# RobertPincus/i3rc-monte-carlo-model

Measured on AMD Instinct MI355X. Metric: photons/s (whole node) + achieved HBM GB/s, I3RC step-cloud 1e8 photons, higher is better.
Workload: dtype f32

## Files before the change

i3rc-monte-carlo-model_amd/binding.py:

```python
import ctypes as C
import os

import numpy as np

from . import build as _build

fp = C.POINTER(C.c_float)
dp = C.POINTER(C.c_double)
ip = C.POINTER(C.c_int32)
lp = C.POINTER(C.c_int64)
up = C.POINTER(C.c_uint32)

MAX_COMPONENTS = 255
MAX_DIRECTIONS = 255
NUM_COUNTERS = 16
COUNTER_NAMES = ["photons", "dropped", "cellSteps", "scatterings", "surfaceHits", "exitsTop", "roulette",
                 "shadowSteps", "tracerCalls", "rngDraws", "raysSkipped"]

SYMBOLS = [
    "i3rc_hip_create", "i3rc_hip_destroy", "i3rc_hip_last_error", "i3rc_hip_set_inverse_table",
    "i3rc_hip_set_forward_tables", "i3rc_hip_set_params", "i3rc_hip_set_surface", "i3rc_hip_set_directions",
    "i3rc_hip_get_tally_layout", "i3rc_hip_bind_tally_buffer", "i3rc_hip_set_stream", "i3rc_hip_use_own_stream", "i3rc_hip_zero_tallies",
    "i3rc_hip_launch_batch", "i3rc_hip_run_batches", "i3rc_hip_run_batches_moments", "i3rc_hip_get_moments_layout", "i3rc_hip_compute_batch", "i3rc_hip_expect_batches", "i3rc_hip_run_replay", "i3rc_hip_trace_rays", "i3rc_hip_synchronize",
    "i3rc_hip_fetch_tallies", "i3rc_hip_normalise", "i3rc_hip_last_kernel_ms", "i3rc_hip_kernel_ms_history", "i3rc_hip_set_tuning", "i3rc_hip_force_general_kernel", "i3rc_hip_select_kernel", "i3rc_hip_set_light_threshold", "i3rc_hip_set_launch_limit",
    "i3rc_hip_set_batch_fusion", "i3rc_hip_select_grid_place", "i3rc_hip_has_column_records", "i3rc_hip_column_records", "i3rc_hip_column_records_base", "i3rc_hip_lds_plan", "i3rc_hip_lds_plan_words", "i3rc_hip_set_lds_tallies", "i3rc_hip_last_kernel_name", "i3rc_hip_last_plan", "i3rc_hip_timed_launch_count", "i3rc_hip_philox_blocks", "i3rc_hip_arith_check", "i3rc_hip_find_index", "i3rc_hip_surface_reflectance", "i3rc_hip_device_count", "i3rc_hip_version",
    "i3rc_hip_set_level_fluxes", "i3rc_hip_get_level_flux_layout", "i3rc_hip_normalise_level_fluxes",
    "i3rc_hip_set_actinic_flux", "i3rc_hip_get_actinic_flux_layout", "i3rc_hip_normalise_actinic_flux",
    "i3rc_hip_set_path_lengths", "i3rc_hip_get_path_length_layout", "i3rc_hip_normalise_path_lengths",
    "i3rc_hip_set_path_histogram", "i3rc_hip_get_path_histogram_layout", "i3rc_hip_normalise_path_histogram",
    "i3rc_hip_problem_facts", "i3rc_hip_plan_launch",
    "i3rc_hip_run_batches_diagnostic_moments", "i3rc_hip_get_diagnostic_moments_layout", "i3rc_hip_diagnostic_moments_layout_words",
    "i3rc_hip_set_path_spectrum", "i3rc_hip_get_path_moments_layout", "i3rc_hip_path_moments_layout_words", "i3rc_hip_run_batches_path_moments",
]


class Params(C.Structure):
    _fields_ = [
        ("surfaceAlbedo", C.c_float), ("useSurfaceBDRF", C.c_int32), ("useRayTracing", C.c_int32),
        ("useRussianRoulette", C.c_int32), ("useHybridPhaseFunsForIntenCalcs", C.c_int32),
# ... 151 lines not shown
    L.i3rc_hip_fetch_tallies.argtypes = [H, dp]
    L.i3rc_hip_normalise.argtypes = [H, dp, fp, fp, fp, fp, fp, fp]
    L.i3rc_hip_last_kernel_ms.argtypes = [H, fp]
    L.i3rc_hip_kernel_ms_history.argtypes = [H, C.c_int, fp]
    if hasattr(L, "i3rc_hip_last_kernel_name"):
        L.i3rc_hip_last_kernel_name.argtypes = [H]
        L.i3rc_hip_timed_launch_count.argtypes = [H]
        L.i3rc_hip_timed_launch_count.restype = C.c_int64
        L.i3rc_hip_last_kernel_name.restype = C.c_char_p
    if hasattr(L, "i3rc_hip_last_plan"):
        L.i3rc_hip_last_plan.argtypes = [H, ip, C.c_int]
    L.i3rc_hip_set_tuning.argtypes = [H, C.c_int, C.c_int]
    L.i3rc_hip_force_general_kernel.argtypes = [H, C.c_int]
    L.i3rc_hip_select_kernel.argtypes = [H, C.c_int]
    L.i3rc_hip_set_light_threshold.argtypes = [H, C.c_int]
    L.i3rc_hip_set_launch_limit.argtypes = [H, C.c_int64]
    if hasattr(L, "i3rc_hip_set_batch_fusion"):
        L.i3rc_hip_set_batch_fusion.argtypes = [H, C.c_int]
    if hasattr(L, "i3rc_hip_select_grid_place"):
        L.i3rc_hip_select_grid_place.argtypes = [H, C.c_int]
        L.i3rc_hip_has_column_records.argtypes = [H]
        L.i3rc_hip_column_records.argtypes = [C.c_int, C.c_int, C.c_int, fp, up]
    if hasattr(L, "i3rc_hip_column_records_base"):
        L.i3rc_hip_column_records_base.argtypes = [C.c_int, C.c_int, C.c_int, fp, up, fp]
    if hasattr(L, "i3rc_hip_lds_plan"):
        L.i3rc_hip_lds_plan.argtypes = [ip, ip]
        L.i3rc_hip_set_lds_tallies.argtypes = [H, C.c_int]
    if hasattr(L, "i3rc_hip_lds_plan_words"):
        L.i3rc_hip_lds_plan_words.argtypes = [ip, C.c_int, ip, C.c_int]
    L.i3rc_hip_philox_blocks.argtypes = [H, C.c_uint32, C.c_uint32, C.c_int64, C.c_int64, C.c_int, up, fp]
# ... 45 lines not shown
```

i3rc-monte-carlo-model_amd/csrc/i3rc_hip.hip:

```cpp
#include "../../include/i3rc_hip.h"

#include <hip/hip_runtime.h>
#include <ctime>
#include <map>
#include <utility>

#include "kernels.hpp"
#include "tally_block.hpp"
#include "launch_plan.hpp"

using namespace i3rc;

namespace {

thread_local std::string g_createError;

bool poison() { static const bool on = std::getenv("I3RC_POISON") != nullptr; return on; }

bool tracing() { static const bool on = std::getenv("I3RC_TRACE") != nullptr; return on; }
double trace_ms() {
  timespec ts; clock_gettime(CLOCK_MONOTONIC, &ts);
  static const double t0 = ts.tv_sec * 1e3 + ts.tv_nsec * 1e-6;
  return ts.tv_sec * 1e3 + ts.tv_nsec * 1e-6 - t0;
}


struct DevBuf {
  void *p = nullptr;
  size_t bytes = 0;
  DevBuf() = default;
  DevBuf(const DevBuf &) = delete;
  DevBuf &operator=(const DevBuf &) = delete;
  ~DevBuf() { if (p) (void)hipFree(p); }
  hipError_t upload(const void *src, size_t n) {
    hipError_t e = alloc(n);
    if (e != hipSuccess) return e;
    if (n) e = hipMemcpy(p, src, n, hipMemcpyHostToDevice);
    return e;
  }
  hipError_t alloc(size_t n) {
    if (p) { (void)hipFree(p); p = nullptr; }
    bytes = n;
    hipError_t e = hipMalloc(&p, n ? n : 4);
    if (e == hipSuccess && poison()) {
      e = hipMemset(p, 0xFF, n ? n : 4);
      if (e == hipSuccess) e = hipDeviceSynchronize();
    }
    return e;
  }
};

}

struct i3rc_hip_integrator : ProblemFacts {
  int device = 0;
  std::vector<float> xE, yE, zE;
  std::vector<double> areaFrac, layerDepth;
  DevBuf dxE, dyE, dzE, dExt, dCum, dSsa, dPf;
  DevBuf dCellRec;
  DevBuf dExtBrick;
  DevBuf dClearMap;
  DevBuf dColRec;
  DevBuf dColBase;
  bool compDirty = true;
  std::vector<DevBuf> dInv, dInvCos, dFwd, dFwdOrig;
  DevBuf dComp;
  DevBuf dXs, dYs, dBrdf;
  float brdf0 = 0.f;
  DevBuf dDir;
  DevBuf dBins;
  std::vector<float> binEdges;

  i3rc_tally_layout layout{};
  TallyView view{};
  DevBuf ownTally;
  double *tally = nullptr;
  DevBuf workCounter;
  DevBuf srcBuf[5];

  struct PipeSlot {
    hipStream_t stream = nullptr;
    DevBuf tally, counter, excess;
    double *pinned = nullptr;
    hipEvent_t done = nullptr;
// ... 522 lines not shown
  int64_t *const out[4] = {binUp, binPathUp, binDown, binPathDown};
  for (int f = 0; f < 4; ++f)
    if (out[f]) *out[f] = on ? block + path_bin_field(f, h->pathBins) : -1;
  if (nBins) *nBins = on ? h->pathBins : 0;
  if (total) *total = h->layout.total;
  return 0;
}

int i3rc_hip_set_tuning(i3rc_hip_integrator *h, int evThreshold, int blocksPerCU) {
  if (!h) return 1;
  drop_lookahead(h);
  if (evThreshold >= 0 && evThreshold <= 64) h->evThreshold = evThreshold;
  if (blocksPerCU >= 0 && blocksPerCU <= 8) h->blocksPerCU = blocksPerCU;
  return 0;
}

int i3rc_hip_set_light_threshold(i3rc_hip_integrator *h, int lanes) {
  if (!h) return 1;
  drop_lookahead(h);
  if (lanes < 0 || lanes > 64) return h->fail("i3rc_hip_set_light_threshold: need 1..64 lanes (0 = default)");
  h->lightThreshold = lanes;
  return 0;
}

int i3rc_hip_set_launch_limit(i3rc_hip_integrator *h, int64_t photons) {
  if (!h) return 1;
  drop_lookahead(h);
  if (photons < 0) return h->fail("i3rc_hip_set_launch_limit: negative limit");
  h->launchLimit = photons;
  return 0;
// ... 128 lines not shown
  std::memset(&P, 0, sizeof(P));
  P.nx = h->nx; P.ny = h->ny; P.nz = h->nz; P.ncomp = h->ncomp;
  P.xyRegular = h->xyRegular; P.zRegular = h->zRegular;
  P.x0 = h->xE.front(); P.xMax = h->xE.back();
  P.y0 = h->yE.front(); P.yMax = h->yE.back();
  P.z0 = h->zE.front(); P.zMax = h->zE.back();
  P.deltaX = h->xE[1] - h->xE[0]; P.deltaY = h->yE[1] - h->yE[0]; P.deltaZ = h->zE[1] - h->zE[0];
  P.xE = (const float *)h->dxE.p; P.yE = (const float *)h->dyE.p; P.zE = (const float *)h->dzE.p;
  P.colRec = (const uint2 *)h->dColRec.p; P.colBase = (const float *)h->dColBase.p;
  P.extBrick = (const float *)h->dExtBrick.p;
  P.bsx = h->bsx; P.bsy = h->bsy; P.bsz = h->bsz; P.nbx = h->nbx; P.nbxy = h->nbx * h->nby;
  P.clearMap = (const uint32_t *)h->dClearMap.p; P.clearShift = h->clearShift; P.clearNx = h->clearNx;
  P.totalExt = (const float *)h->dExt.p;
}

int make_problem(i3rc_hip_integrator *h, const LaunchDecision &d, DevProblem &P, hipStream_t stream, double *tally) {
  fill_geometry(h, P);
  if (d.place != GRID_COLUMNS && d.place != GRID_COLBASE) P.colRec = nullptr;
  if (d.place != GRID_COLBASE) P.colBase = nullptr;
  if (d.place != GRID_BRICKS) P.extBrick = nullptr;
  P.cumExt = (const float *)h->dCum.p; P.ssa = (const float *)h->dSsa.p;
  P.pfIndex = (const int32_t *)h->dPf.p;
  P.cellRec = (const uint4 *)h->dCellRec.p;
  if (h->compDirty) {
    if (hipStreamSynchronize(stream) != hipSuccess ||
        hipMemcpy(h->dComp.p, h->comp.data(), sizeof(CompTables) * h->ncomp, hipMemcpyHostToDevice) != hipSuccess)
      return h->fail("copying the component table descriptors failed");
    h->compDirty = false;
  }
  P.comp = (const CompTables *)h->dComp.p;
  P.comp0 = h->comp[0];
// ... 4 lines not shown
  P.useRayTracing = traced(*h) ? 1 : 0; P.useRR = h->params.useRussianRoulette;
  P.nDir = h->nDir; P.useHybrid = h->params.useHybridPhaseFunsForIntenCalcs;
  P.numOrdersOrig = h->params.numOrdersOrigPhaseFunIntenCalcs; P.useRRI = h->params.useRussianRouletteForIntensity;
  P.limitContrib = h->params.limitIntensityContributions; P.zetaMin = h->params.zetaMin;
  P.maxContrib = h->params.maxIntensityContribution; P.maxExt = h->maxExt;
  P.dirCos = (const float *)h->dDir.p;
  if (h->extra == EXTRA_PATH_BINS && h->nDir == 0) P.dirCos = (const float *)h->dBins.p;
  P.uniformSsa = h->uniformSsa; P.uniformPf = h->uniformPf;
  P.eventFlags = event_flags(P.uniformSsa, P.uniformPf, P.useBDRF != 0, P.albedo, P.useRR != 0);
  P.tally = tally;
  const TallyView &V = h->view;
  P.oUp = (int)V.fluxUp; P.oDown = (int)V.fluxDown; P.oAbs = (int)V.fluxAbsorbed; P.oVol = (int)V.volumeAbsorption;
  P.oInt = (int)V.intensityByComponent; P.oExc = (int)V.intensityExcess; P.oCnt = (int)V.counters;
  P.rayQueueCap = d.rayQueueCap;
  P.ldsTallies = d.ldsTallies; P.ldsVolume = d.ldsVolume; P.ldsIntensity = d.ldsIntensity; P.ldsGrid = d.ldsGrid | (d.ldsBins ? kLdsGridBinSums : 0);
  return 0;
}

__global__ void __launch_bounds__(256) absorbed_columns_kernel(double *blocks, long long stride, int oAbs, int oVol, int ncol, int nz) {
  const int col = (int)(blockIdx.x * 256 + threadIdx.x);
  if (col >= ncol) return;
  double *const blk = blocks + (size_t)blockIdx.y * stride;
  double s = 0.0;
  for (int k = 0; k < nz; ++k) s += blk[oVol + (size_t)k * ncol + col];
  blk[oAbs + col] = s;
}
int absorbed_columns(i3rc_hip_integrator *h, hipStream_t stream, double *blocks, int nBlocks, long long stride) {
  if (!h->absorbing || nBlocks < 1) return 0;
  const int ncol = h->nx * h->ny;
  for (int first = 0; first < nBlocks; first += 65535) {
    const int n = std::min(65535, nBlocks - first);
// ... 23 lines not shown
  for (int k = 0; k < 5; ++k) if (!arrs[k]) return h->fail("explicit photon stream: null array");
  for (int64_t i = 0; i < n; ++i) {
    const float mu = src->mu[i];
    if (!(std::fabs(mu) <= 1.f) || !(std::fabs(mu) > FLT_MIN)) return h->fail("setIllumination: solarMu out of bounds");
    if (!(src->x[i] >= 0.f && src->x[i] <= 1.f) || !(src->y[i] >= 0.f && src->y[i] <= 1.f) || !(src->z[i] >= 0.f && src->z[i] <= 1.f))
      return h->fail("setIllumination: photon position out of bounds (relative positions lie in [0, 1])");
    if (!std::isfinite(src->phi[i])) return h->fail("setIllumination: solarAzimuth out of bounds");
  }
  for (int k = 0; k < 5; ++k) {
    HIPCHK(h, h->srcBuf[k].upload(arrs[k], sizeof(float) * (size_t)n));
    *dst[k] = (const float *)h->srcBuf[k].p;
  }
  return 0;
}

int prepare_launch(i3rc_hip_integrator *h, const StreamKind &s, const i3rc_source *src, int64_t n, hipStream_t stream, double *tally,
                   Launch &L, RunArgs &A) {
  L.d = plan_launch(*h, EnvKnobs::process(), {s, src->kind});
  if (!L.d.refusal.empty() && L.d.early) return h->fail(L.d.refusal);
  if (upload_source(h, src, n, A)) return 1;
  if (!L.d.refusal.empty()) return h->fail(L.d.refusal);
  return make_problem(h, L.d, L.P, stream, tally);
}

using Kernel = void (*)(DevProblem, RunArgs, int, int);
struct KernelEntry {
  KernelKey key;
  Kernel fn;
  const char *name;
};

template <class Rng>
constexpr const char *rng_name() {
  if constexpr (Rng::kExtra == EXTRA_LEVELS) return "PhiloxLevelStream";
  else if constexpr (Rng::kExtra == EXTRA_TRACKS) return "PhiloxTrackStream";
  else if constexpr (Rng::kExtra == EXTRA_PATHS) return "PhiloxPathStream";
  else if constexpr (Rng::kExtra == EXTRA_PATH_BINS) return "PhiloxBinStream";
// ... 132 lines not shown
        int tx = 1, ty = 8;
        for (int cx = 2; cx <= 8; cx *= 2)
          if ((double)h->nx / cx + (double)h->ny / (8 / cx) < (double)h->nx / tx + (double)h->ny / ty) { tx = cx; ty = 8 / cx; }
        hipLaunchKernelGGL(slab_count_kernel, dim3(kSlabSortBlocks), dim3(256), 0, stream, A.seed0, A.seed1, A.firstPhoton, A.nPhotons, span,
                           tx, ty, (unsigned *)sb.blockCounts.p);
        hipLaunchKernelGGL(slab_scan_kernel, dim3(1), dim3(8), 0, stream, (int)kSlabSortBlocks, (const unsigned *)sb.blockCounts.p,
                           (SlabMeta *)sb.meta.p, (unsigned *)sb.blockBase.p);
        hipLaunchKernelGGL(slab_fill_kernel, dim3(kSlabSortBlocks), dim3(256), 0, stream, A.seed0, A.seed1, A.firstPhoton, A.nPhotons, span,
                           tx, ty, (const unsigned *)sb.blockBase.p, (uint32_t *)sb.ids.p);
        HIPCHK(h, hipGetLastError());
        B.slabIds = (const uint32_t *)sb.ids.p; B.slabMeta = (SlabMeta *)sb.meta.p;
      }
    }
    static const long long chunkMax = std::max(64ll, env_int("I3RC_CHUNK_MAX", 256));
    B.chunk = (int)std::min<long long>(chunkMax, std::max<long long>(64, A.nPhotons / (blocks * (threads / 64) * 8)));
    HIPCHK(h, hipMemsetAsync(A.workCounter, 0, sizeof(unsigned long long), stream));
    return 0;
  });
  if (rc) return 1;
  return absorbed_columns(h, stream, L.P.tally, 1, 0);
}

__global__ void __launch_bounds__(256) reduce_replicas_kernel(const double *blocks, double *out, long long nBlocksOut, int R, long long stride) {
  const long long i = (long long)blockIdx.x * 256 + threadIdx.x;
  if (i >= nBlocksOut * stride) return;
  const long long b = i / stride, e = i - b * stride;
  const double *src = blocks + (size_t)b * R * stride + e;
  double v = 0.0;
  for (int r = 0; r < R; ++r) v += src[(size_t)r * stride];
  out[i] = v;
// ... 1073 lines not shown
```

i3rc-monte-carlo-model_amd/csrc/kernels.hpp:

```cpp
#pragma once
#include <cstddef>
#include "tally_block.hpp"
#include "event_flags.hpp"
#include "pass_decision.hpp"
#include "tracer.hpp"
#include "tuning.hpp"

namespace i3rc {

enum LaneState { ST_TRACE = 0, ST_EVENT = 1, ST_DROPPED = 2, ST_NEW = 3, ST_DONE = 4,
                 ST_EXIT = 5 };

struct WaveCounters {
  uint32_t photons = 0, dropped = 0, steps = 0, scat = 0, surf = 0, top = 0, roul = 0, shadow = 0, calls = 0;
};
struct NestedCounters { uint32_t shadow = 0, calls = 0; };
struct LanePairs {
  uint32_t word = 0u;
  __device__ __forceinline__ void add(bool low, bool high) { word += (low ? 1u : 0u) + (high ? 1u << 16 : 0u); }
  __device__ __forceinline__ uint32_t low() const { return word & 0xffffu; }
  __device__ __forceinline__ uint32_t high() const { return word >> 16; }
  static __device__ __forceinline__ bool about_to_overflow(LanePairs a, LanePairs b) { return ((a.word | b.word) & ((1u << 15) | (1u << 31))) != 0u; }
};

// ... 336 lines not shown
};
template <class Rng>
constexpr bool has_start_store(bool intensity, bool general, int grid, bool multi) {
  return !Rng::kReplay && !Rng::kBatched && Rng::kExtra == EXTRA_NONE && !intensity && !general && !multi && grid != GRID_BRICKS;
}
template <class Rng, bool INTENSITY, bool GENERAL, int GRID, bool TBL = false, bool DIRECT = false, bool MULTI = false>
__global__ void __launch_bounds__(TBL ? 1024 : 256, (planned_waves<Rng, INTENSITY, GENERAL, GRID, TBL, MULTI>()))
photon_kernel(const DevProblem P, const RunArgs A, const int evThreshold, const int lightThreshold) {
  extern __shared__ __attribute__((aligned(16))) float smem[];
  Lds L;
  constexpr bool STORE = has_start_store<Rng>(INTENSITY, GENERAL, GRID, MULTI);
  constexpr bool FLAGS = STORE && I3RC_EVENT_FLAGS != 0;
  constexpr int STEP_FORM = !STORE ? 0 : (I3RC_STEP_BIASED_ADDRESS ? STEP_BIASED : 0) | (I3RC_STEP_STATE_SELECTS ? STEP_MASKS : 0) |
                                         (I3RC_STEP_COLD_ERROR ? STEP_COLD_ERROR : 0) | (I3RC_STEP_ADVANCE_MASKS ? STEP_ADVANCE_MASKS : 0);
  constexpr bool ROULETTE_BIT = FLAGS && I3RC_ROULETTE_FLAG != 0;
  constexpr bool PASS_BITS = STORE && I3RC_PASS_DECISION != 0;
  constexpr bool TURN_WORD = STORE && I3RC_TURN_ALL_WORD != 0;
  constexpr bool TURN_RANGE = STORE && I3RC_TURN_STATE_RANGE != 0;
  constexpr int kStDropped = TURN_RANGE ? (int)ST_DONE : (int)ST_DROPPED, kStDone = TURN_RANGE ? (int)ST_DROPPED : (int)ST_DONE;
  static_assert(!TURN_RANGE || (ST_NEW == 3 && kStDropped == 4 && ST_EXIT == 5 && kStDone < ST_NEW && ST_TRACE < ST_NEW && ST_EVENT < ST_NEW),
                "the turnover states are the states from ST_NEW on");
  constexpr bool CHAIN = !GENERAL && Rng::kBatched && INTENSITY && !DIRECT && GRID == GRID_BRICKS;
  constexpr bool ZERO_IS_SLOW = GENERAL || CHAIN;
  lds_float *startSlots = nullptr;
  constexpr bool TRACK = Rng::kExtra == EXTRA_TRACKS;
  lds_f64 *trackSums = nullptr;
  constexpr bool BINS = Rng::kExtra == EXTRA_PATH_BINS;
  BinTable bins;
  {
    const LdsPlan lp = lds_plan(P, INTENSITY && !Rng::kReplay, DIRECT, GRID, INTENSITY, TBL ? 16 : 4, 0, STORE);
// ... 228 lines not shown
      uint32_t draws = rng.take_used();
#pragma unroll
      for (int off = 32; off > 0; off >>= 1) draws += (uint32_t)__shfl_xor((int)draws, off, 64);
      if ((threadIdx.x & 63) == 0) {
        double *const c = counter_block(res.batch);
        const uint32_t v[8] = {wc.steps, wc.scat, wc.surf, wc.top, wc.roul, wc.shadow, wc.scat + wc.surf + wc.top + wc.calls, draws};
        const int at[8] = {I3RC_CNT_CELL_STEPS, I3RC_CNT_SCATTERINGS, I3RC_CNT_SURFACE_HITS, I3RC_CNT_EXITS_TOP, I3RC_CNT_ROULETTE,
                           I3RC_CNT_SHADOW_STEPS, I3RC_CNT_TRACER_CALLS, I3RC_CNT_RNG_DRAWS};
#pragma unroll
        for (int k = 0; k < 8; ++k)
          if (v[k] != 0u) unsafeAtomicAdd(c + at[k], (double)v[k]);
        if (raysSkipped != 0u) unsafeAtomicAdd(c + I3RC_CNT_RAYS_SKIPPED, (double)raysSkipped);
      }
      raysSkipped = 0u;
    }
    if (!BATCHED && (threadIdx.x & 63) == 0) {
      const uint32_t calls = STORE ? wc.scat + wc.surf + wc.top + wc.dropped : wc.calls;
      const uint32_t c[9] = {wc.photons, wc.dropped, wc.steps, wc.scat, wc.surf, wc.top, wc.roul, wc.shadow, calls};
      const ColdArgs ka = cold_args();
      double *const counters = ka->P.tally + ka->P.oCnt;
#pragma unroll
      for (int k = 0; k < 9; ++k)
        if (c[k] != 0u) unsafeAtomicAdd(counters + k, (double)c[k]);
    }
    wc = WaveCounters();
  };
  auto make_ray = [&](const auto &Px, const auto &Ax, int info, float inX, float inY, float inZ, uint32_t photonLo, uint32_t photonHi,
                      uint32_t eventBlock, uint32_t batch, int dIdx, float &rayWord, float &normOut, float &tauFreeOut, float &targetOut) -> bool {
    const int comp = EventInfo::component(info);
    const float uz = L.dirCos[3 * dIdx + 2];
    float norm;
    if (comp < 1) norm = 1.0f / kPi;
    else {
// ... 344 lines not shown
          }
          if constexpr (LANE_COUNTS) {
            const bool leaves = isNew && mine >= 0 && mineBatch != rng.batch && (accSteps | accA.word | accB.word | rng.used) != 0u;
            if (__ballot(leaves) != 0ull) flush_lanes(leaves);
          }
          if (isNew) {
            if (mine < 0) st = kStDone;
            else rng.start((uint64_t)(Ae.firstPhoton + mine), mineBatch);
          }
        }
      } else if constexpr (STORE) {
        if (newMask != 0ull) {
          int need = __popcll(newMask);
          int rank = lanes_below(newMask);
          long long mine = -1;
          for (;;) {
            const int take = need < startAvail ? need : startAvail;
            if (isNew && mine < 0 && rank >= 0 && rank < take) {
              mine = res.next - startAvail + rank;
              const StartSlot::Words s = StartSlot::load(startSlots + kStartWords * ((unsigned)mine & (unsigned)(kStartSlots - 1)));
              r.x = s.x; r.y = s.y; r.ix = s.ix; r.iy = s.iy; r.target = s.depth;
            }
            startAvail -= take;
            wc.photons += (unsigned)take;
            need -= take; rank -= take;
            if (need == 0) break;
            long long end = startState.end();
            if (res.next >= end) {
              if (end >= cold_args()->A.nPhotons) break;
              const unsigned refilled = (unsigned)__builtin_amdgcn_readfirstlane(startState.w[WaveStartState::kRefills]) + 1u;
              startState.w[WaveStartState::kRefills] = (int)refilled;
              if ((refilled & 3u) == 0u || wc.steps > 0x40000000u) flush_counters();
              else adapt_thresholds();
              res.refill();
              end = res.end;
              startState.save_end(end);
              if (res.next >= end) break;
            }
            const long long left = end - res.next;
            const int n = left < (long long)kStartSlots ? (int)left : kStartSlots;
            {
              const long long i = res.next + (long long)(threadIdx.x & 63);
              const Philox4 o = rng.first_block_of((uint64_t)(cold_args()->A.firstPhoton + i));
              const float px = u32_to_unit_float(o.v[0]);
              float py = u32_to_unit_float(o.v[1]);
#ifdef I3RC_EXPERIMENT_SLAB
              py *= 0.125f;
// ... 5 lines not shown
                const auto &Px = cold_args()->P;
                x = Px.x0 + px * (Px.xMax - Px.x0);
                ci = min((int)exact_div(x - Px.x0, Px.deltaX, refined_rcp(Px.deltaX)) + 1, Px.nx);
                if (fabsf(L.xE[ci] - x) < spacingf(x)) ci = ci + 1;
                ci = ci == Px.nx + 1 ? 1 : ci;
              }
              {
                const auto &Py = cold_args()->P;
                y = Py.y0 + py * (Py.yMax - Py.y0);
                cj = min((int)exact_div(y - Py.y0, Py.deltaY, refined_rcp(Py.deltaY)) + 1, Py.ny);
                if (fabsf(L.yE[cj] - y) < spacingf(y)) cj = cj + 1;
                cj = cj == Py.ny + 1 ? 1 : cj;
              }
              StartSlot::store(startSlots + kStartWords * ((unsigned)i & (unsigned)(kStartSlots - 1)), x, y, ci, cj, depth);
            }
            __builtin_amdgcn_wave_barrier();
            res.next += n;
            startAvail = n;
          }
          if (isNew) {
            if (mine < 0) st = kStDone;
            else RngInit<Rng>::start(rng, Ae, mine);
          }
        }
      } else
      if (newMask != 0ull) {
        int need = __popcll(newMask);
        int rank = lanes_below(newMask);
        long long mine = -1;
        long long avail = res.end - res.next;
        const bool slabs = SLABS && Ae.slabIds != nullptr;
        if (avail < (long long)need && (slabs ? res.end >= 0 : res.end < Ae.nPhotons)) {
          if (isNew && rank < (int)avail) mine = res.next + rank;
          wc.photons += (unsigned)avail;
          need -= (int)avail;
          rank -= (int)avail;
          if ((++refills & 3u) == 0u || wc.steps > 0x40000000u || wc.shadow > 0x40000000u) flush_counters();
// ... 458 lines not shown
  r.dx = dir[3 * i]; r.dy = dir[3 * i + 1]; r.dz = dir[3 * i + 2];
  r.ix = idx[3 * i]; r.iy = idx[3 * i + 1]; r.iz = idx[3 * i + 2];
  r.set_direction(L);
  r.acc = 0.0f;
  const bool hasTarget = target[i] >= 0.0f;
  r.target = target[i];
  int ns = 0;
  StepResult s;
  do { ns++; s = trace_step<GRID, CLEARMAP>(P, L, r, hasTarget); } while (s == STEP_CONTINUE && ns < (1 << 24));
  pos[3 * i] = r.x; pos[3 * i + 1] = r.y; pos[3 * i + 2] = r.z;
  idx[3 * i] = r.ix; idx[3 * i + 1] = r.iy; idx[3 * i + 2] = r.iz;
  tau[i] = r.acc;
  steps[i] = ns;
}

__global__ void arith_check_kernel(long long n, const float *num, const float *den, unsigned long long *mismatch) {
  const long long i = (long long)blockIdx.x * blockDim.x + threadIdx.x;
  if (i >= n) return;
  const float a = num[i], b = den[i];
  const float q = exact_div(a, b, refined_rcp(b)), qRef = a / b;
  if (__float_as_uint(q) != __float_as_uint(qRef)) atomicAdd(&mismatch[0], 1ull);
  const float x = fabsf(a);
  if (__float_as_uint(exact_sqrt(x)) != __float_as_uint(sqrtf(x))) atomicAdd(&mismatch[1], 1ull);
}

__global__ void find_index_kernel(int n, const float *table, long long m, const float *values, const int32_t *firstGuess, int32_t *out) {
  const long long i = (long long)blockIdx.x * blockDim.x + threadIdx.x;
  if (i >= m) return;
  out[i] = find_index(values[i], [table](int k) { return table[k - 1]; }, n, firstGuess ? firstGuess[i] : 0);
}
// ... 27 lines not shown
```

i3rc-monte-carlo-model_amd/csrc/launch_plan.hpp:

```cpp
#pragma once

#include <algorithm>
#include <cfloat>
#include <cmath>
#include <cstdio>
#include <cstdlib>
#include <cstring>
#include <string>
#include <vector>

#include "kernels.hpp"
#include "tally_block.hpp"

namespace i3rc {

inline bool env_on(const char *name) { const char *v = std::getenv(name); return !(v && std::atoi(v) == 0); }
inline long long env_int(const char *name, long long dflt) { const char *v = std::getenv(name); return v ? std::atoll(v) : dflt; }
inline bool env_pair(const char *name, int &a, int &b) { const char *v = std::getenv(name); return v && std::sscanf(v, "%d,%d", &a, &b) == 2; }

struct EnvKnobs {
  bool columns = true;
  bool ldsTallies = true;
  bool tableLds = true;
  int plainPlaces = 11;
  int fusedPlaces = 11;
  bool direct = true;
  bool cellRecords = true;
  static const EnvKnobs &process() {
    static const EnvKnobs k{env_on("I3RC_COLUMNS"), env_on("I3RC_LDS_TALLIES"), env_on("I3RC_TABLE_LDS"), (int)env_int("I3RC_TABLE_LDS_PLACES", 11),
                            (int)env_int("I3RC_FUSED_TABLE_LDS_PLACES", 11), env_on("I3RC_DIRECT"), env_on("I3RC_CELL_RECORDS")};
    return k;
  }
};

struct ProblemFacts {
  int nx = 0, ny = 0, nz = 0, ncomp = 0, nDir = 0;
  int xyRegular = 0, zRegular = 0;
  float maxExt = 0.f;
  bool empty = false;
  bool absorbing = false;
  float uniformSsa = -1.f;
  int uniformPf = 0;
  int cellRecBytes = 0;
  bool colRecords = false;
  bool colBase = false;
// ... 295 lines not shown
```

i3rc-monte-carlo-model_amd/csrc/tuning.hpp:

```cpp
#pragma once

#ifndef I3RC_RADIANCE_WAVES
#define I3RC_RADIANCE_WAVES 5
#endif
#ifndef I3RC_MIN_WAVES
#define I3RC_MIN_WAVES 5
#endif
#ifndef I3RC_FLUX_WAVES
#define I3RC_FLUX_WAVES 8
#endif
#ifndef I3RC_FUSED_WAVES
#define I3RC_FUSED_WAVES 7
#endif
#ifndef I3RC_MULTI_WAVES
#define I3RC_MULTI_WAVES 4
#endif

#ifndef I3RC_MERGE_ABSORPTION
#define I3RC_MERGE_ABSORPTION 1
#endif
#ifndef I3RC_CELL_RECORD_READS
#define I3RC_CELL_RECORD_READS 1
#endif

// ... 39 lines not shown
#ifndef I3RC_PASS_DECISION
#define I3RC_PASS_DECISION 1
#endif
#ifndef I3RC_TURN_STATE_RANGE
#define I3RC_TURN_STATE_RANGE 1
#endif
#ifndef I3RC_TURN_ALL_WORD
#define I3RC_TURN_ALL_WORD 1
#endif
#ifndef I3RC_ROULETTE_FLAG
#define I3RC_ROULETTE_FLAG 1
#endif
#ifndef I3RC_STEP_ADVANCE_MASKS
#define I3RC_STEP_ADVANCE_MASKS 1
#endif
#ifndef I3RC_PHOTON_STEP_AHEAD
#define I3RC_PHOTON_STEP_AHEAD 64
#endif
#ifndef I3RC_EXPAND_BATCH
#define I3RC_EXPAND_BATCH 64
#endif
#ifndef I3RC_DIRECT_ENTER
#define I3RC_DIRECT_ENTER 96
#endif
#ifndef I3RC_DIRECT_LEAVE
#define I3RC_DIRECT_LEAVE 24
#endif

#ifndef I3RC_EVTHR_SLOPE_FLUX
#define I3RC_EVTHR_SLOPE_FLUX 2.0f
// ... 11 lines not shown
```

i3rc-monte-carlo-model_amd/host.py:

```python
import ctypes as C

import numpy as np

from . import binding as B
from .binding import I3RCError, f32, pf
from .phasefunctions import PI_MCRT, PhaseFunction, PhaseFunctionTable, hybrid_phase_functions, libm_f32, spacing

r32 = np.float32

DEFAULT_MIN_TABLE_SIZE = 9001


def _directional(solarMu, solarAzimuth):
    s = B.Source()
    s.kind, s.solarMu, s.solarAzimuth = 0, solarMu, solarAzimuth
    return s


class RandomNumberSequence:

    def __init__(self, seed):
        if np.isscalar(seed):
            seed = (int(seed), 0)
        seed = tuple(int(s) & 0xFFFFFFFF for s in seed)
# ... 522 lines not shown
        self._check(self._lib.i3rc_hip_set_lds_tallies(self._h, 1 if on else 0), "set_lds_tallies")

    def kernel_ms(self):
        ms = C.c_float(0)
        self._check(self._lib.i3rc_hip_last_kernel_ms(self._h, C.byref(ms)), "kernel_ms")
        return float(ms.value)

    def timed_launches(self):
        return int(self._lib.i3rc_hip_timed_launch_count(self._h))

    def kernel_name(self):
        if not hasattr(self._lib, "i3rc_hip_last_kernel_name"):
            return "?"
        return self._lib.i3rc_hip_last_kernel_name(self._h).decode()

    def last_plan(self):
        names = B.PLAN_NAMES + ([B.PLAN_BIN_NAME] if self.pathHistogramEdges is not None else [])
        out = (C.c_int32 * len(names))()
        self._check(self._lib.i3rc_hip_last_plan(self._h, out, len(names)), "last_plan")
        return dict(zip(names, (int(v) for v in out)))

    def kernel_ms_history(self, n):
        ms = np.zeros(n, np.float32)
        self._check(self._lib.i3rc_hip_kernel_ms_history(self._h, int(n), pf(ms)), "kernel_ms_history")
        return ms

    def reportResults(self, levelFluxUp=False, levelFluxDown=False, actinicFlux=False, pathLengthUp=False, pathLengthSquaredUp=False,
                      pathLengthDown=False, pathLengthSquaredDown=False, pathHistogramUp=False, pathHistogramPathUp=False,
                      pathHistogramDown=False, pathHistogramPathDown=False):
        r = self._results
# ... 18 lines not shown
        if "intensity" in r:
            out["intensity"] = r["intensity"]
            out["meanIntensity"] = r["intensity"].sum(axis=(1, 2), dtype=np.float32) / ncol
        if levelFluxUp:
            out["levelFluxUp"] = r["levelFluxUp"]
        if levelFluxDown:
            out["levelFluxDown"] = r["levelFluxDown"]
        if actinicFlux:
            out["actinicFlux"] = r["actinicFlux"]
        for k in paths + bins:
            out[k] = r[k]
        return out

    KERNELS = {"auto": 0, "general": 1, "lane": 2, "ring": 3}

    def set_tuning(self, evThreshold=0, blocksPerCU=0, forceGeneral=None, kernel=None, lightThreshold=None):
        self._check(self._lib.i3rc_hip_set_tuning(self._h, int(evThreshold), int(blocksPerCU)), "set_tuning")
        if forceGeneral is not None:
            self._check(self._lib.i3rc_hip_force_general_kernel(self._h, int(bool(forceGeneral))), "set_tuning")
        if kernel is not None:
            self._check(self._lib.i3rc_hip_select_kernel(self._h, self.KERNELS[kernel]), "set_tuning")
        if lightThreshold is not None:
            self._check(self._lib.i3rc_hip_set_light_threshold(self._h, int(lightThreshold)), "set_tuning")

    GRID_PLACES = {"auto": 0, "linear": 1, "bricks": 2, "columns": 3}

    def select_grid_place(self, place):
        self._check(self._lib.i3rc_hip_select_grid_place(self._h, self.GRID_PLACES[place]), "select_grid_place")

    def has_column_records(self):
        return bool(self._lib.i3rc_hip_has_column_records(self._h))

    def trace_rays(self, direction, pos, idx, target=None):
        d, p = f32(direction).reshape(-1, 3).copy(), f32(pos).reshape(-1, 3).copy()
        i = np.ascontiguousarray(idx, np.int32).reshape(-1, 3).copy()
        n = len(d)
        t = np.full(n, -1.0, np.float32) if target is None else f32(target).copy()
        tau, steps = np.zeros(n, np.float32), np.zeros(n, np.int32)
# ... 101 lines not shown
```

include/i3rc_hip.h:

```cpp
#ifndef I3RC_HIP_H
#define I3RC_HIP_H
#include <stddef.h>
#include <stdint.h>

#ifdef __cplusplus
extern "C" {
#endif

typedef struct i3rc_hip_integrator i3rc_hip_integrator;

#define I3RC_MAX_COMPONENTS 255
#define I3RC_MAX_DIRECTIONS 255

typedef struct i3rc_params {
  float   surfaceAlbedo;
  int32_t useSurfaceBDRF;
  int32_t useRayTracing;
  int32_t useRussianRoulette;
  int32_t useHybridPhaseFunsForIntenCalcs;
  int32_t numOrdersOrigPhaseFunIntenCalcs;
  int32_t useRussianRouletteForIntensity;
  float   zetaMin;
  int32_t limitIntensityContributions;
  float   maxIntensityContribution;
// ... 151 lines not shown
int i3rc_hip_normalise(const i3rc_hip_integrator *h, const double *hostTallies,
                       float *fluxUp, float *fluxDown, float *fluxAbsorbed, float *volumeAbsorption,
                       float *intensity, float *intensityByComponent);

int i3rc_hip_last_kernel_ms(i3rc_hip_integrator *h, float *ms);
int i3rc_hip_kernel_ms_history(i3rc_hip_integrator *h, int n, float *ms);

int64_t i3rc_hip_timed_launch_count(const i3rc_hip_integrator *h);

const char *i3rc_hip_last_kernel_name(const i3rc_hip_integrator *h);

int i3rc_hip_last_plan(const i3rc_hip_integrator *h, int32_t *out, int n);

int i3rc_hip_set_tuning(i3rc_hip_integrator *h, int evThreshold, int blocksPerCU);
int i3rc_hip_set_light_threshold(i3rc_hip_integrator *h, int lanes);

int i3rc_hip_set_launch_limit(i3rc_hip_integrator *h, int64_t photons);

int i3rc_hip_set_batch_fusion(i3rc_hip_integrator *h, int mode);

enum { I3RC_KERNEL_AUTO = 0, I3RC_KERNEL_GENERAL = 1, I3RC_KERNEL_LANE = 2, I3RC_KERNEL_RING = 3 };
int i3rc_hip_select_kernel(i3rc_hip_integrator *h, int variant);
int i3rc_hip_force_general_kernel(i3rc_hip_integrator *h, int on);

enum { I3RC_GRID_AUTO = 0, I3RC_GRID_LINEAR = 1, I3RC_GRID_BRICKS = 2, I3RC_GRID_COLUMNS = 3 };
int i3rc_hip_select_grid_place(i3rc_hip_integrator *h, int place);
int i3rc_hip_has_column_records(const i3rc_hip_integrator *h);
int i3rc_hip_column_records(int nx, int ny, int nz, const float *totalExt, uint32_t *records);
int i3rc_hip_column_records_base(int nx, int ny, int nz, const float *totalExt, uint32_t *records, float *base);

// ... 29 lines not shown
```

Before: 4.720 billion.

## Precompute per-column optical-depth table to jump photons' first flight directly

For overhead-sun solar sources, a device kernel builds a per-column cumulative optical-depth table once per problem. At photon launch, each lane binary-searches this table to place the photon directly at its first interaction layer or the surface, instead of stepping through cells one by one. Lanes too close to a cell edge fall back to normal tracing. Skipped steps are folded into the counters through ballots, and the start chunk size is capped. In exchange the change adds table memory, extra launch-time logic and LDS traffic, and a correctness dependency on the table matching the traced path.

```diff
diff --git a/i3rc-monte-carlo-model_amd/binding.py b/i3rc-monte-carlo-model_amd/binding.py
--- a/i3rc-monte-carlo-model_amd/binding.py
+++ b/i3rc-monte-carlo-model_amd/binding.py
@@ -22,7 +22,7 @@
     "i3rc_hip_set_forward_tables", "i3rc_hip_set_params", "i3rc_hip_set_surface", "i3rc_hip_set_directions",
     "i3rc_hip_get_tally_layout", "i3rc_hip_bind_tally_buffer", "i3rc_hip_set_stream", "i3rc_hip_use_own_stream", "i3rc_hip_zero_tallies",
     "i3rc_hip_launch_batch", "i3rc_hip_run_batches", "i3rc_hip_run_batches_moments", "i3rc_hip_get_moments_layout", "i3rc_hip_compute_batch", "i3rc_hip_expect_batches", "i3rc_hip_run_replay", "i3rc_hip_trace_rays", "i3rc_hip_synchronize",
-    "i3rc_hip_fetch_tallies", "i3rc_hip_normalise", "i3rc_hip_last_kernel_ms", "i3rc_hip_kernel_ms_history", "i3rc_hip_set_tuning", "i3rc_hip_force_general_kernel", "i3rc_hip_select_kernel", "i3rc_hip_set_light_threshold", "i3rc_hip_set_launch_limit",
+    "i3rc_hip_fetch_tallies", "i3rc_hip_normalise", "i3rc_hip_last_kernel_ms", "i3rc_hip_kernel_ms_history", "i3rc_hip_set_tuning", "i3rc_hip_force_general_kernel", "i3rc_hip_select_kernel", "i3rc_hip_set_light_threshold", "i3rc_hip_set_first_flight_table", "i3rc_hip_last_first_flight", "i3rc_hip_set_launch_limit",
     "i3rc_hip_set_batch_fusion", "i3rc_hip_select_grid_place", "i3rc_hip_has_column_records", "i3rc_hip_column_records", "i3rc_hip_column_records_base", "i3rc_hip_lds_plan", "i3rc_hip_lds_plan_words", "i3rc_hip_set_lds_tallies", "i3rc_hip_last_kernel_name", "i3rc_hip_last_plan", "i3rc_hip_timed_launch_count", "i3rc_hip_philox_blocks", "i3rc_hip_arith_check", "i3rc_hip_find_index", "i3rc_hip_surface_reflectance", "i3rc_hip_device_count", "i3rc_hip_version",
     "i3rc_hip_set_level_fluxes", "i3rc_hip_get_level_flux_layout", "i3rc_hip_normalise_level_fluxes",
     "i3rc_hip_set_actinic_flux", "i3rc_hip_get_actinic_flux_layout", "i3rc_hip_normalise_actinic_flux",
@@ -204,6 +204,9 @@
     L.i3rc_hip_force_general_kernel.argtypes = [H, C.c_int]
     L.i3rc_hip_select_kernel.argtypes = [H, C.c_int]
     L.i3rc_hip_set_light_threshold.argtypes = [H, C.c_int]
+    if hasattr(L, "i3rc_hip_set_first_flight_table"):
+        L.i3rc_hip_set_first_flight_table.argtypes = [H, C.c_int]
+        L.i3rc_hip_last_first_flight.argtypes = [H]
     L.i3rc_hip_set_launch_limit.argtypes = [H, C.c_int64]
     if hasattr(L, "i3rc_hip_set_batch_fusion"):
         L.i3rc_hip_set_batch_fusion.argtypes = [H, C.c_int]
diff --git a/i3rc-monte-carlo-model_amd/csrc/first_flight.hpp b/i3rc-monte-carlo-model_amd/csrc/first_flight.hpp
--- /dev/null
+++ b/i3rc-monte-carlo-model_amd/csrc/first_flight.hpp
@@ -0,0 +1,61 @@
+#pragma once
+
+#include <stdint.h>
+
+#if defined(__HIP__) || defined(__HIPCC__)
+#define I3RC_FLIGHT_FN __host__ __device__ __forceinline__
+#else
+#define I3RC_FLIGHT_FN inline
+#endif
+
+namespace i3rc {
+
+constexpr unsigned kFirstFlight = 16u;
+
+constexpr int kFlightIyShift = 11, kFlightCodeShift = 22;
+constexpr int kFlightMaxColumns = 2047, kFlightMaxLayers = 1022;
+constexpr int kFlightBottom = 0, kFlightNotLanded = 1023;
+I3RC_FLIGHT_FN int flight_pack(int ix, int iy, int code) { return ix | (iy << kFlightIyShift) | (code << kFlightCodeShift); }
+I3RC_FLIGHT_FN int flight_ix(int word) { return word & ((1 << kFlightIyShift) - 1); }
+I3RC_FLIGHT_FN int flight_iy(int word) { return (word >> kFlightIyShift) & ((1 << kFlightIyShift) - 1); }
+I3RC_FLIGHT_FN int flight_code(int word) { return (int)((uint32_t)word >> kFlightCodeShift); }
+
+I3RC_FLIGHT_FN bool first_flight_eligible(bool storeLaunch, int srcKind, float solarDx, float solarDy, float solarDz, int startLayer, int nx, int ny, int nz,
+                                          bool tableExists) {
+  return storeLaunch && srcKind == 0 && solarDx == 0.0f && solarDy == 0.0f && solarDz == -1.0f && startLayer >= 1 && startLayer <= nz &&
+         nx <= kFlightMaxColumns && ny <= kFlightMaxColumns && nz <= kFlightMaxLayers && tableExists;
+}
+
+struct FlightLanding {
+  int steps;
+  int layer;
+  float z;
+};
+template <class Table, class Ext, class Edges, class Divide>
+I3RC_FLIGHT_FN FlightLanding first_flight_landing(const Table &A, const Ext &ext, const Edges &zE, float zStart, int startLayer, float dz, float t,
+                                                  const Divide &divide) {
+  int lo = 1, hi = startLayer + 1;
+  while (lo < hi) {
+    const int mid = (int)((unsigned)(lo + hi) >> 1);
+    if (A(mid) > t) hi = mid; else lo = mid + 1;
+  }
+  FlightLanding o;
+  o.steps = lo > startLayer ? startLayer : lo;
+  o.layer = lo > startLayer ? 0 : startLayer - lo + 1;
+  o.z = 0.0f;
+  if (o.layer != 0) {
+    const float rest = t - A(lo - 1);
+    const float part = divide(rest, ext(o.layer));
+    const float face = lo == 1 ? zStart : zE[o.layer];
+    o.z = face + part * dz;
+  }
+  return o;
+}
+
+I3RC_FLIGHT_FN bool first_flight_lands(float z, float surfaceZ, float zMax) {
+  union { float f; uint32_t u; } b;
+  b.f = z;
+  return (b.u & 0x7f800000u) != 0x7f800000u && z > surfaceZ && z < zMax;
+}
+
+}
diff --git a/i3rc-monte-carlo-model_amd/csrc/i3rc_hip.hip b/i3rc-monte-carlo-model_amd/csrc/i3rc_hip.hip
--- a/i3rc-monte-carlo-model_amd/csrc/i3rc_hip.hip
+++ b/i3rc-monte-carlo-model_amd/csrc/i3rc_hip.hip
@@ -38,6 +38,7 @@
     if (n) e = hipMemcpy(p, src, n, hipMemcpyHostToDevice);
     return e;
   }
+  void release() { if (p) { (void)hipFree(p); p = nullptr; } bytes = 0; }
   hipError_t alloc(size_t n) {
     if (p) { (void)hipFree(p); p = nullptr; }
     bytes = n;
@@ -68,6 +69,11 @@
   DevBuf dXs, dYs, dBrdf;
   float brdf0 = 0.f;
   DevBuf dDir;
+  DevBuf dFlight;
+  int flightState = 0;
+  int flightLayer = 0;
+  bool flightOn = true;
+  bool lastLanded = false;
   DevBuf dBins;
   std::vector<float> binEdges;
 
@@ -620,6 +626,15 @@
   if (blocksPerCU >= 0 && blocksPerCU <= 8) h->blocksPerCU = blocksPerCU;
   return 0;
 }
+
+int i3rc_hip_set_first_flight_table(i3rc_hip_integrator *h, int on) {
+  if (!h) return 1;
+  drop_lookahead(h);
+  h->flightOn = on != 0;
+  return 0;
+}
+
+int i3rc_hip_last_first_flight(const i3rc_hip_integrator *h) { return h && h->lastLanded ? 1 : 0; }
 
 int i3rc_hip_set_light_threshold(i3rc_hip_integrator *h, int lanes) {
   if (!h) return 1;
@@ -778,7 +793,8 @@
   P.totalExt = (const float *)h->dExt.p;
 }
 
-int make_problem(i3rc_hip_integrator *h, const LaunchDecision &d, DevProblem &P, hipStream_t stream, double *tally) {
+int first_flight(i3rc_hip_integrator *h, const LaunchDecision &d, DevProblem &P, const RunArgs &A, hipStream_t stream);
+int make_problem(i3rc_hip_integrator *h, const LaunchDecision &d, DevProblem &P, const RunArgs &A, hipStream_t stream, double *tally) {
   fill_geometry(h, P);
   if (d.place != GRID_COLUMNS && d.place != GRID_COLBASE) P.colRec = nullptr;
   if (d.place != GRID_COLBASE) P.colBase = nullptr;
@@ -813,7 +829,7 @@
   P.oInt = (int)V.intensityByComponent; P.oExc = (int)V.intensityExcess; P.oCnt = (int)V.counters;
   P.rayQueueCap = d.rayQueueCap;
   P.ldsTallies = d.ldsTallies; P.ldsVolume = d.ldsVolume; P.ldsIntensity = d.ldsIntensity; P.ldsGrid = d.ldsGrid | (d.ldsBins ? kLdsGridBinSums : 0);
-  return 0;
+  return first_flight(h, d, P, A, stream);
 }
 
 __global__ void __launch_bounds__(256) absorbed_columns_kernel(double *blocks, long long stride, int oAbs, int oVol, int ncol, int nz) {
@@ -867,13 +883,65 @@
   return 0;
 }
 
+constexpr size_t kFlightTableMax = (size_t)256 << 20;
+hipError_t make_flight_table(i3rc_hip_integrator *h, const DevProblem &P, hipStream_t stream, int &layer, bool &fit) {
+#if I3RC_FIRST_FLIGHT_TABLE != 0
+  const size_t ncol = (size_t)P.nx * P.ny;
+  DevBuf info;
+  int words[2] = {0, 1};
+  hipError_t e = h->dFlight.alloc(sizeof(float) * ncol * (size_t)(P.nz + 1));
+  if (e == hipSuccess) e = info.alloc(sizeof(words));
+  if (e == hipSuccess) e = hipMemsetAsync(info.p, 0, sizeof(words), stream);
+  if (e == hipSuccess) {
+    const size_t lds = sizeof(float) * (size_t)(P.nx + P.ny + P.nz + 3);
+    hipLaunchKernelGGL(first_flight_table_kernel, dim3((unsigned)((ncol + 255) / 256)), dim3(256), lds, stream, P, (float *)h->dFlight.p, (int *)info.p);
+    e = hipGetLastError();
+  }
+  if (e == hipSuccess) e = hipMemcpyAsync(words, info.p, sizeof(words), hipMemcpyDeviceToHost, stream);
+  if (e == hipSuccess) e = hipStreamSynchronize(stream);
+  if (e != hipSuccess) { h->dFlight.release(); return e; }
+  layer = words[0]; fit = words[1] == 0;
+  return hipSuccess;
+#else
+  (void)h; (void)P; (void)stream; (void)layer; (void)fit;
+  return hipSuccess;
+#endif
+}
+int first_flight(i3rc_hip_integrator *h, const LaunchDecision &d, DevProblem &P, const RunArgs &A, hipStream_t stream) {
+  h->lastLanded = false;
+#if I3RC_FIRST_FLIGHT_TABLE != 0
+  const bool store = d.startStore && P.nDir == 0;
+  if (!h->flightOn || !EnvKnobs::process().firstFlight) return 0;
+  if (!first_flight_eligible(store, A.srcKind, A.solarDx, A.solarDy, A.solarDz, 1, P.nx, P.ny, P.nz, true)) return 0;
+  if (h->flightState == 0 && P.totalExt != nullptr) {
+    const size_t bytes = sizeof(float) * (size_t)P.nx * P.ny * (size_t)(P.nz + 1);
+    if (bytes > kFlightTableMax) h->flightState = 2;
+    else {
+      bool fit = false;
+      if (make_flight_table(h, P, stream, h->flightLayer, fit) == hipSuccess) {
+        h->flightState = fit ? 1 : 2;
+        if (!fit) h->dFlight.release();
+      } else (void)hipGetLastError();
+    }
+  }
+  if (first_flight_eligible(store, A.srcKind, A.solarDx, A.solarDy, A.solarDz, h->flightLayer, P.nx, P.ny, P.nz, h->flightState == 1)) {
+    P.eventFlags |= kFirstFlight;
+    h->lastLanded = true;
+    P.dirCos = (const float *)h->dFlight.p;
+  }
+#else
+  (void)h; (void)d; (void)P; (void)A; (void)stream;
+#endif
+  return 0;
+}
+
 int prepare_launch(i3rc_hip_integrator *h, const StreamKind &s, const i3rc_source *src, int64_t n, hipStream_t stream, double *tally,
                    Launch &L, RunArgs &A) {
   L.d = plan_launch(*h, EnvKnobs::process(), {s, src->kind});
   if (!L.d.refusal.empty() && L.d.early) return h->fail(L.d.refusal);
   if (upload_source(h, src, n, A)) return 1;
   if (!L.d.refusal.empty()) return h->fail(L.d.refusal);
-  return make_problem(h, L.d, L.P, stream, tally);
+  return make_problem(h, L.d, L.P, A, stream, tally);
 }
 
 using Kernel = void (*)(DevProblem, RunArgs, int, int);
@@ -1036,6 +1104,7 @@
     }
     static const long long chunkMax = std::max(64ll, env_int("I3RC_CHUNK_MAX", 256));
     B.chunk = (int)std::min<long long>(chunkMax, std::max<long long>(64, A.nPhotons / (blocks * (threads / 64) * 8)));
+    if ((L.P.eventFlags & kFirstFlight) != 0u) B.chunk = std::min(B.chunk, 1 << 16);
     HIPCHK(h, hipMemsetAsync(A.workCounter, 0, sizeof(unsigned long long), stream));
     return 0;
   });
diff --git a/i3rc-monte-carlo-model_amd/csrc/kernels.hpp b/i3rc-monte-carlo-model_amd/csrc/kernels.hpp
--- a/i3rc-monte-carlo-model_amd/csrc/kernels.hpp
+++ b/i3rc-monte-carlo-model_amd/csrc/kernels.hpp
@@ -3,6 +3,7 @@
 #include "tally_block.hpp"
 #include "event_flags.hpp"
 #include "pass_decision.hpp"
+#include "first_flight.hpp"
 #include "tracer.hpp"
 #include "tuning.hpp"
 
@@ -374,6 +375,7 @@
   constexpr int STEP_FORM = !STORE ? 0 : (I3RC_STEP_BIASED_ADDRESS ? STEP_BIASED : 0) | (I3RC_STEP_STATE_SELECTS ? STEP_MASKS : 0) |
                                          (I3RC_STEP_COLD_ERROR ? STEP_COLD_ERROR : 0) | (I3RC_STEP_ADVANCE_MASKS ? STEP_ADVANCE_MASKS : 0);
   constexpr bool ROULETTE_BIT = FLAGS && I3RC_ROULETTE_FLAG != 0;
+  constexpr bool FLIGHT = STORE && I3RC_FIRST_FLIGHT_TABLE != 0;
   constexpr bool PASS_BITS = STORE && I3RC_PASS_DECISION != 0;
   constexpr bool TURN_WORD = STORE && I3RC_TURN_ALL_WORD != 0;
   constexpr bool TURN_RANGE = STORE && I3RC_TURN_STATE_RANGE != 0;
@@ -632,9 +634,15 @@
       }
       raysSkipped = 0u;
     }
+    uint32_t landedSteps = 0u;
+    if constexpr (FLIGHT) {
+      const unsigned word = (unsigned)__builtin_amdgcn_readfirstlane(startState.w[WaveStartState::kRefills]);
+      landedSteps = word >> 2;
+      startState.w[WaveStartState::kRefills] = (int)(word & 3u);
+    }
     if (!BATCHED && (threadIdx.x & 63) == 0) {
       const uint32_t calls = STORE ? wc.scat + wc.surf + wc.top + wc.dropped : wc.calls;
-      const uint32_t c[9] = {wc.photons, wc.dropped, wc.steps, wc.scat, wc.surf, wc.top, wc.roul, wc.shadow, calls};
+      const uint32_t c[9] = {wc.photons, wc.dropped, FLIGHT ? wc.steps + landedSteps : wc.steps, wc.scat, wc.surf, wc.top, wc.roul, wc.shadow, calls};
       const ColdArgs ka = cold_args();
       double *const counters = ka->P.tally + ka->P.oCnt;
 #pragma unroll
@@ -1009,12 +1017,26 @@
           int need = __popcll(newMask);
           int rank = lanes_below(newMask);
           long long mine = -1;
+          bool flightLaunch = false;
+          if constexpr (FLIGHT) flightLaunch = (Pe.eventFlags & kFirstFlight) != 0u;
           for (;;) {
             const int take = need < startAvail ? need : startAvail;
             if (isNew && mine < 0 && rank >= 0 && rank < take) {
               mine = res.next - startAvail + rank;
+              if constexpr (FLIGHT) {
+                if (flightLaunch) {
+                  const lds_float *const slot = startSlots + kStartWords * ((unsigned)mine & (unsigned)(kStartSlots - 1));
+                  const int cellWord = __float_as_int(slot[StartSlot::kCell]);
+                  r.x = slot[StartSlot::kX]; r.y = slot[StartSlot::kY]; r.target = slot[StartSlot::kDepth];
+                  r.ix = flight_ix(cellWord); r.iy = flight_iy(cellWord); r.iz = flight_code(cellWord);
+                } else {
+                  const StartSlot::Words s = StartSlot::load(startSlots + kStartWords * ((unsigned)mine & (unsigned)(kStartSlots - 1)));
+                  r.x = s.x; r.y = s.y; r.ix = s.ix; r.iy = s.iy; r.target = s.depth;
+                }
+              } else {
               const StartSlot::Words s = StartSlot::load(startSlots + kStartWords * ((unsigned)mine & (unsigned)(kStartSlots - 1)));
               r.x = s.x; r.y = s.y; r.ix = s.ix; r.iy = s.iy; r.target = s.depth;
+              }
             }
             startAvail -= take;
             wc.photons += (unsigned)take;
@@ -1023,9 +1045,10 @@
             long long end = startState.end();
             if (res.next >= end) {
               if (end >= cold_args()->A.nPhotons) break;
-              const unsigned refilled = (unsigned)__builtin_amdgcn_readfirstlane(startState.w[WaveStartState::kRefills]) + 1u;
+              unsigned refilled = (unsigned)__builtin_amdgcn_readfirstlane(startState.w[WaveStartState::kRefills]) + 1u;
+              if constexpr (FLIGHT) refilled = ((refilled - 1u) & ~3u) | (refilled & 3u);
               startState.w[WaveStartState::kRefills] = (int)refilled;
-              if ((refilled & 3u) == 0u || wc.steps > 0x40000000u) flush_counters();
+              if ((refilled & 3u) == 0u || wc.steps > 0x40000000u || (FLIGHT && refilled > 0x80000000u)) flush_counters();
               else adapt_thresholds();
               res.refill();
               end = res.end;
@@ -1061,6 +1084,43 @@
               }
               StartSlot::store(startSlots + kStartWords * ((unsigned)i & (unsigned)(kStartSlots - 1)), x, y, ci, cj, depth);
             }
+            if constexpr (FLIGHT) {
+              if (flightLaunch) {
+                asm volatile("" ::: "memory");
+                lds_float *const slot = startSlots + kStartWords * (((unsigned)res.next + (threadIdx.x & 63u)) & (unsigned)(kStartSlots - 1));
+                const int cell = __float_as_int(slot[StartSlot::kCell]);
+                const int ci = cell & ((1 << StartSlot::kIyShift) - 1), cj = (int)((unsigned)cell >> StartSlot::kIyShift);
+                unsigned long long nearMask;
+                {
+                  const float x = slot[StartSlot::kX], y = slot[StartSlot::kY];
+                  nearMask = __ballot((fabsf(L.xE[ci] - x) <= two_spacingf(x)) | (fabsf(L.yE[cj] - y) <= two_spacingf(y)));
+                }
+                const auto &Pf = cold_args()->P;
+                const float depth = slot[StartSlot::kDepth];
+                const float *const table = Pf.dirCos;
+                const unsigned row = (__umul24((unsigned)(cj - 1), (unsigned)Pf.nx) + (unsigned)(ci - 1)) * (unsigned)(Pf.nz + 1);
+                const int layer0 = __builtin_amdgcn_readfirstlane(startState.w[WaveStartState::kLayer]);
+                const float zTop = Pf.zMax;
+                const float zFrom = Pf.z0 + (1.0f - spacingf(1.0f)) * (zTop - Pf.z0);
+                const FlightLanding f = first_flight_landing(
+                    [table, row](int k) { return *(const float *)((const char *)table + ((row + (unsigned)k) << 2)); }, [&](int iz) { return cell_extinction<GRID>(Pf, L, ci, cj, iz); }, L.zE, zFrom,
+                    layer0, -1.0f, depth, [](float rest, float e) {
+                      float part = exact_div(rest, e, refined_rcp(e));
+                      if (__builtin_expect(e < 1e-20f, 0)) part = rest / e;
+                      return part;
+                    });
+                const bool bottom = f.layer == kFlightBottom;
+                const bool lands = !__builtin_amdgcn_inverse_ballot_w64(nearMask) && (bottom || first_flight_lands(f.z, surfaceZ, zTop));
+                slot[StartSlot::kCell] = __int_as_float(flight_pack(ci, cj, lands ? f.layer : kFlightNotLanded));
+                if (lands && !bottom) slot[StartSlot::kDepth] = f.z;
+                const uint32_t mySteps = lands && (int)(threadIdx.x & 63) < n ? (uint32_t)f.steps : 0u;
+                uint32_t landedSteps = 0u;
+                static_assert(kFlightMaxLayers < (1 << 10), "a lane's landed steps fit ten bits");
+#pragma unroll
+                for (int b = 0; b < 10; ++b) landedSteps += (uint32_t)__popcll(__ballot(((mySteps >> b) & 1u) != 0u)) << b;
+                startState.w[WaveStartState::kRefills] = (int)((unsigned)__builtin_amdgcn_readfirstlane(startState.w[WaveStartState::kRefills]) + (landedSteps << 2));
+              }
+            }
             __builtin_amdgcn_wave_barrier();
             res.next += n;
             startAvail = n;
@@ -1068,6 +1128,24 @@
           if (isNew) {
             if (mine < 0) st = kStDone;
             else RngInit<Rng>::start(rng, Ae, mine);
+          }
+          if constexpr (FLIGHT) {
+            if (flightLaunch) {
+              const bool taken = isNew && mine >= 0;
+              const bool landed = taken && r.iz != kFlightNotLanded;
+              const bool scatters = taken && (unsigned)(r.iz - 1) < (unsigned)(kFlightNotLanded - 1);
+              wc.scat += (unsigned)__popcll(__ballot(scatters));
+              if (landed) {
+                rng.block = 1u;
+                rng.count_draws(3u);
+                r.dx = Ae.solarDx; r.dy = Ae.solarDy; r.dz = Ae.solarDz;
+                order = 0;
+                w = 1.0f;
+                r.z = r.target; r.target = 0.0f;
+                st = scatters ? ST_EVENT : (blackSurface ? ST_EXIT : ST_EVENT);
+                wantEvent = scatters;
+              }
+            }
           }
         }
       } else
@@ -1556,6 +1634,48 @@
   steps[i] = ns;
 }
 
+#if I3RC_FIRST_FLIGHT_TABLE != 0
+__global__ void __launch_bounds__(256) first_flight_table_kernel(const DevProblem P, float *table, int *info) {
+  extern __shared__ __attribute__((aligned(16))) float smem[];
+  Lds L;
+  L.xE = (lds_float *)smem; L.yE = L.xE + P.nx + 1; L.zE = L.yE + P.ny + 1;
+  L.tUp = L.tDown = L.tVol = nullptr; L.dirCos = nullptr; L.ext = nullptr;
+  for (int i = threadIdx.x; i <= P.nx; i += blockDim.x) L.xE[i] = P.xE[i];
+  for (int i = threadIdx.x; i <= P.ny; i += blockDim.x) L.yE[i] = P.yE[i];
+  for (int i = threadIdx.x; i <= P.nz; i += blockDim.x) L.zE[i] = P.zE[i];
+  __syncthreads();
+  const int col = (int)(blockIdx.x * blockDim.x + threadIdx.x);
+  if (col >= P.nx * P.ny) return;
+  const float zStart = P.z0 + (1.0f - spacingf(1.0f)) * (P.zMax - P.z0);
+  int izStart = 1;
+  find_z<true>(P, L, zStart, izStart);
+  if (col == 0) info[0] = izStart;
+  float *const row = table + (size_t)col * (size_t)(P.nz + 1);
+  bool bad = izStart < 1 || izStart > P.nz;
+  float last = 0.0f;
+  row[0] = 0.0f;
+  int k = 1;
+  if (!bad) {
+    const int ix = col % P.nx + 1, iy = col / P.nx + 1;
+    Ray r;
+    r.x = 0.5f * (L.xE[ix - 1] + L.xE[ix]); r.y = 0.5f * (L.yE[iy - 1] + L.yE[iy]); r.z = zStart;
+    r.dx = 0.0f; r.dy = 0.0f; r.dz = -1.0f;
+    r.ix = ix; r.iy = iy; r.iz = izStart;
+    r.set_direction(L);
+    r.acc = 0.0f; r.target = kHuge;
+    for (; k <= izStart; ++k) {
+      const StepResult s = trace_step_lazy<GRID_GLOBAL>(P, L, r, true);
+      const bool ok = s == (k < izStart ? STEP_CONTINUE : STEP_EXIT) && r.iz == izStart - k && r.ix == ix && r.iy == iy && r.acc >= last && r.acc < kHuge;
+      if (!ok) { bad = true; break; }
+      last = r.acc;
+      row[k] = last;
+    }
+  }
+  for (; k <= P.nz; ++k) row[k] = last;
+  if (bad) atomicOr(&info[1], 1);
+}
+#endif
+
 __global__ void arith_check_kernel(long long n, const float *num, const float *den, unsigned long long *mismatch) {
   const long long i = (long long)blockIdx.x * blockDim.x + threadIdx.x;
   if (i >= n) return;
diff --git a/i3rc-monte-carlo-model_amd/csrc/launch_plan.hpp b/i3rc-monte-carlo-model_amd/csrc/launch_plan.hpp
--- a/i3rc-monte-carlo-model_amd/csrc/launch_plan.hpp
+++ b/i3rc-monte-carlo-model_amd/csrc/launch_plan.hpp
@@ -26,9 +26,10 @@
   int fusedPlaces = 11;
   bool direct = true;
   bool cellRecords = true;
+  bool firstFlight = true;
   static const EnvKnobs &process() {
     static const EnvKnobs k{env_on("I3RC_COLUMNS"), env_on("I3RC_LDS_TALLIES"), env_on("I3RC_TABLE_LDS"), (int)env_int("I3RC_TABLE_LDS_PLACES", 11),
-                            (int)env_int("I3RC_FUSED_TABLE_LDS_PLACES", 11), env_on("I3RC_DIRECT"), env_on("I3RC_CELL_RECORDS")};
+                            (int)env_int("I3RC_FUSED_TABLE_LDS_PLACES", 11), env_on("I3RC_DIRECT"), env_on("I3RC_CELL_RECORDS"), env_on("I3RC_FIRST_FLIGHT_TABLE")};
     return k;
   }
 };
diff --git a/i3rc-monte-carlo-model_amd/csrc/tuning.hpp b/i3rc-monte-carlo-model_amd/csrc/tuning.hpp
--- a/i3rc-monte-carlo-model_amd/csrc/tuning.hpp
+++ b/i3rc-monte-carlo-model_amd/csrc/tuning.hpp
@@ -77,6 +77,9 @@
 #ifndef I3RC_STEP_ADVANCE_MASKS
 #define I3RC_STEP_ADVANCE_MASKS 1
 #endif
+#ifndef I3RC_FIRST_FLIGHT_TABLE
+#define I3RC_FIRST_FLIGHT_TABLE 1
+#endif
 #ifndef I3RC_PHOTON_STEP_AHEAD
 #define I3RC_PHOTON_STEP_AHEAD 64
 #endif
diff --git a/i3rc-monte-carlo-model_amd/host.py b/i3rc-monte-carlo-model_amd/host.py
--- a/i3rc-monte-carlo-model_amd/host.py
+++ b/i3rc-monte-carlo-model_amd/host.py
@@ -560,6 +560,9 @@
             return "?"
         return self._lib.i3rc_hip_last_kernel_name(self._h).decode()
 
+    def first_flight_landed(self):
+        return hasattr(self._lib, "i3rc_hip_last_first_flight") and bool(self._lib.i3rc_hip_last_first_flight(self._h))
+
     def last_plan(self):
         names = B.PLAN_NAMES + ([B.PLAN_BIN_NAME] if self.pathHistogramEdges is not None else [])
         out = (C.c_int32 * len(names))()
@@ -608,7 +611,7 @@
 
     KERNELS = {"auto": 0, "general": 1, "lane": 2, "ring": 3}
 
-    def set_tuning(self, evThreshold=0, blocksPerCU=0, forceGeneral=None, kernel=None, lightThreshold=None):
+    def set_tuning(self, evThreshold=0, blocksPerCU=0, forceGeneral=None, kernel=None, lightThreshold=None, firstFlightTable=None):
         self._check(self._lib.i3rc_hip_set_tuning(self._h, int(evThreshold), int(blocksPerCU)), "set_tuning")
         if forceGeneral is not None:
             self._check(self._lib.i3rc_hip_force_general_kernel(self._h, int(bool(forceGeneral))), "set_tuning")
@@ -616,6 +619,8 @@
             self._check(self._lib.i3rc_hip_select_kernel(self._h, self.KERNELS[kernel]), "set_tuning")
         if lightThreshold is not None:
             self._check(self._lib.i3rc_hip_set_light_threshold(self._h, int(lightThreshold)), "set_tuning")
+        if firstFlightTable is not None:
+            self._check(self._lib.i3rc_hip_set_first_flight_table(self._h, int(bool(firstFlightTable))), "set_tuning")
 
     GRID_PLACES = {"auto": 0, "linear": 1, "bricks": 2, "columns": 3}
 
diff --git a/include/i3rc_hip.h b/include/i3rc_hip.h
--- a/include/i3rc_hip.h
+++ b/include/i3rc_hip.h
@@ -189,6 +189,8 @@
 
 int i3rc_hip_set_tuning(i3rc_hip_integrator *h, int evThreshold, int blocksPerCU);
 int i3rc_hip_set_light_threshold(i3rc_hip_integrator *h, int lanes);
+int i3rc_hip_set_first_flight_table(i3rc_hip_integrator *h, int on);
+int i3rc_hip_last_first_flight(const i3rc_hip_integrator *h);
 
 int i3rc_hip_set_launch_limit(i3rc_hip_integrator *h, int64_t photons);
 
```

New measurement: 4.827 billion, median of 6. 2.3% higher.
